# m96-chan/PyGPUkit

Hardware: AMD Instinct MI355X
Metric: decode tokens/sec/GPU + prefill TFLOPS (% MFMA peak), Qwen3-0.6B bf16 (higher is better)
Workload: dtype bf16

## Files before the change

### pygpukit_amd/csrc/engine.hip

```cpp

#include "engine_attn.hip.h"
#include "engine_gemv.hip.h"
#include "pkgemm.hip.h"

namespace pgk {

__global__ void embed_kernel(const bf16* embed, const int32_t* tokens, float* h, int H, const int32_t* positions,
                             const float* rope_cos, const float* rope_sin, float* cur_cos, float* cur_sin, int half,
                             int max_seq) {
    const int b = blockIdx.x;
    const bf16* row = embed + (size_t)tokens[b] * H;
    for (int i = threadIdx.x; i < H; i += blockDim.x) h[(size_t)b * H + i] = to_f(row[i]);
    const int pos = min(positions[b], max_seq - 1);
    for (int i = threadIdx.x; i < half; i += blockDim.x) {
        cur_cos[(size_t)b * half + i] = rope_cos[(size_t)pos * half + i];
        cur_sin[(size_t)b * half + i] = rope_sin[(size_t)pos * half + i];
    }
}

__global__ __launch_bounds__(256) void finalize_kernel(unsigned long long* tl, const float* amax_val, const int* amax_idx, int nblk,
                                                       int32_t* tokens, int32_t* positions, int32_t* token_log,
                                                       int32_t* step_counter, int log_width, int log_cap,
                                                       const bf16* embed, float* h, int H, int bump,
                                                       unsigned long long* clk_log, const float* rope_cos,
// ... 836 lines not shown
}

pgk_status pgk_engine_linear_plan(pgk_engine eh, int batch, int max_position, int prefill_n, char* out, size_t n) {
    PGK_REQUIRE(eh && out && n > 0, "pgk_engine_linear_plan: null argument");
    const Engine* e = (const Engine*)eh;
    const auto& c = e->cfg;
    size_t used = 0;
    out[0] = 0;
    auto emit = [&](const char* fmt, auto... args) -> bool {
        const int w = snprintf(out + used, n - used, fmt, args...);
        if (w <= 0 || (size_t)w >= n - used) return false;
        used += (size_t)w;
        return true;
    };
    const int H = c.hidden_size, I = c.intermediate_size, QD = c.num_heads * c.head_dim, NQKV = e->qkv_dim(), V = c.vocab_size;
    if (prefill_n > 0) {
        PGK_REQUIRE(prefill_n <= c.max_seq_len, "pgk_engine_linear_plan: %d tokens outside cache of %d", prefill_n, c.max_seq_len);
        const PrefillChoice p = prefill_choice(e, prefill_n);
        const char* path = p.fp8act ? "fp8act" : (p.pk ? "pk" : (p.ws ? "ws" : "gemm"));
        const int s_qkv = p.ws && !p.pk ? p.s_qkv : 1, s_gu = p.ws && !p.pk ? p.s_gu : 1;
        const int s_o = p.fp8act ? 1 : (p.pk ? (p.carried ? 1 : p.pk_so) : (p.ws ? p.s_o : p.g_so));
        const int s_d = p.fp8act ? 1 : (p.pk ? (p.carried ? 1 : p.pk_sd) : (p.ws ? p.s_d : p.g_sd));
        PGK_REQUIRE(emit("prefill n=%d path=%s ws=%d pk=%d pk_heads=%d carried=%d pkd=%d nvf4=%d fp8act=%d fuse_heads=%d fuse_heads8=%d fuse_sw16=%d fuse_sw8=%d "
                         "s_qkv=%d s_o=%d s_gu=%d s_d=%d\n", prefill_n, path, (int)p.ws, (int)p.pk, (int)p.pk_heads, (int)p.carried, (int)p.pkd, (int)p.nv4,
                         (int)p.fp8act, (int)p.fuse_heads, (int)p.fuse_heads8, (int)p.fuse_sw16, (int)p.fuse_sw8, s_qkv, s_o, s_gu, s_d),
                    "pgk_engine_linear_plan: the plan needs more than %zu bytes", n);
        return PGK_OK;
    }
    PGK_REQUIRE(batch >= 1 && batch <= c.max_batch, "pgk_engine_linear_plan: batch %d outside [1,%d]", batch, c.max_batch);
    PGK_REQUIRE(max_position >= 0 && max_position < c.max_seq_len, "pgk_engine_linear_plan: position %d outside cache of %d", max_position, c.max_seq_len);
    static const char* const forms[] = {"gemv", "batched", "tiled", "packed"};
    const bool short_ctx = step_is_short_at(e, batch, max_position) && e->short_path;
    const bool fp8 = c.weight_format == 1 || c.weight_format == 2;
    const int nw = c.weight_format == 3 ? GEMV_NW_NVF4 : (fp8 ? GEMV_NW_FP8 : GEMV_NW_BF16);
    const char* wname = c.weight_format == 3 ? "nvf4" : (fp8 ? "fp8" : "bf16");
    bool ok = true;
    for (int b0 = 0; b0 < batch && ok;) {
        const ChunkChoice ch = next_chunk(e, batch - b0);
        const AttnFlags af = attn_flags(e, ch.form, ch.m, short_ctx);
        const int M = ch.m;
        if (ch.form == CF_GEMV) {
            const bool partials = af.fused || af.merged;
            const char* act = M >= 4 ? "bf16" : "f32";
            ok = emit("chunk b0=%d m=%d form=gemv act=%s oproj=%s carried=0 normrows=0 attn16=none\n", b0, M, act, af.fused ? "fused" : (af.merged ? "merged" : "own"));
            auto gemv = [&](const char* name, int wnw, const char* wn, const char* pro, bool swiglu, int n_out, int K, int r, int force_grid) {
                if (r == 0) r = gemv_rows(wnw, M, swiglu, n_out, K);
                ok = ok && emit("proj name=%s kernel=fused_gemv m=%d act=%s w=%s pro=%s r=%d c=%d grid=%d n=%d k=%d\n", name, M, act, wn, pro, r,
                                gemv_preload(wnw, r, K), gemv_grid(r, swiglu, n_out, force_grid), n_out, K);
            };
            gemv("qkv", nw, wname, "norm", false, NQKV, H, 0, 0);
            if (!partials) gemv("o", nw, wname, "plain", false, H, QD, 0, 0);
            gemv("gate_up", nw, wname, partials && M <= 2 ? "norm_sum" : "norm", true, I, H, 0, 0);
            gemv("down", nw, wname, "plain", false, H, I, 0, 0);
            gemv("lm_head", GEMV_NW_BF16, "bf16", "norm", false, V, H, 4, e->lm_blocks);
        } else if (ch.form == CF_PACKED) {
            const bool carried = e->packed_resid;
            ok = emit("chunk b0=%d m=%d form=packed act=bf16 oproj=own carried=%d normrows=0 attn16=%s\n", b0, M, carried ? 1 : 0, af.direct ? "direct" : "normrows");
            ok = ok && emit("proj name=qkv kernel=pkgemm splits=1 n=%d k=%d\n", NQKV, H);
            ok = ok && emit("proj name=o kernel=%s splits=%d n=%d k=%d\n", carried ? "pkgemm_resid" : "pkgemm", carried ? 1 : pkgemm_pick_splits(M, H, QD), H, QD);
            ok = ok && emit("proj name=gate_up kernel=pkgemm splits=1 n=%d k=%d\n", 2 * I, H);
            ok = ok && emit("proj name=down kernel=%s splits=%d n=%d k=%d\n", carried ? "pkgemm_resid" : "pkgemm", carried ? 1 : pkgemm_pick_splits(M, H, I), H, I);
            const int rows = mt_rows_per_group(V, true);
            ok = ok && emit("proj name=lm_head kernel=batched_mt w=bf16 rows=%d mp=0 tiles=%d copy=%d grid=%d n=%d k=%d\n", rows, mt_tiles(M),
                            batched_reads_copy(false, rows, e->packed_lm != nullptr) ? 1 : 0, batched_lm_blocks(V), V, H);
        } else {
            const bool tiled = ch.form == CF_TILED;
            ok = emit("chunk b0=%d m=%d form=%s act=bf16 oproj=own carried=0 normrows=%d attn16=%s\n", b0, M, forms[ch.form], tiled ? 1 : 0,
                      af.direct ? "direct" : (tiled ? "normrows" : "none"));
            auto bat = [&](const char* name, bool wfp8, bool logits, bool have_copy, int N, int K) {
                const char* wn = wfp8 ? "fp8" : "bf16";
                if (tiled) {
                    const int rows = mt_rows_per_group(N, logits);
                    ok = ok && emit("proj name=%s kernel=batched_mt w=%s rows=%d mp=0 tiles=%d copy=%d grid=%d n=%d k=%d\n", name, wn, rows, mt_tiles(M),
                                    batched_reads_copy(wfp8, rows, have_copy) ? 1 : 0, logits ? batched_lm_blocks(V) : ceil_div(N, rows), N, K);
                } else if (batched_is_reg(K)) {
                    const int rows = batched_reg_rows(N, logits);
                    ok = ok && emit("proj name=%s kernel=batched_reg w=%s rows=%d mp=0 tiles=1 copy=%d grid=%d n=%d k=%d\n", name, wn, rows,
                                    batched_reads_copy(wfp8, rows, have_copy) ? 1 : 0, logits ? batched_lm_blocks(V) : ceil_div(N, rows), N, K);
                } else {
                    ok = ok && emit("proj name=%s kernel=batched_lds w=%s rows=16 mp=%d tiles=1 copy=0 grid=%d n=%d k=%d\n", name, wn, M <= 8 ? 8 : 16,
                                    logits ? batched_lm_blocks(V) : ceil_div(N, 16), N, K);
                }
            };
// ... 21 lines not shown
```

### pygpukit_amd/csrc/engine_prefill.hip

```cpp

#include "attn_plan.h"
#include "engine_gemv.hip.h"
#include "engine_state.hip.h"
#include "gemm_epilogues.hip.h"
#include "pkgemm.hip.h"

namespace pgk {

pgk_status engine_gemm_nt(const bf16* A, const void* W, const bf16* wscale, bool fp8, void* C, bool accum_f32, int M,
                          int N, int K, hipStream_t st, bool packed = false);
bool engine_gemm_packed_ok(int M, int N, int K);
int wsgemm_pick_splits(int N, int K, bool allow_split);
int engine_gemm_pick_splits(int M, int N, int K);
pgk_status engine_gemm_nt_slabs(const bf16* A, const void* W, float* slabs, int splits, int M, int N, int K, hipStream_t st, bool packed = false);
pgk_status gemm_fp8_nt(const uint8_t* a, const float* sa, const uint8_t* w, const bf16* sw, void* c, bool accum_f32, int M,
                       int N, int K, hipStream_t st);
pgk_status quantize_fp8_rows_bf16(const bf16* x, uint8_t* out, float* scale, int M, int K, hipStream_t st);
bool engine_gemm_qkv_heads_ok(int M, int N, int K);
pgk_status engine_gemm_qkv_heads_nt(const bf16* A, const bf16* W, bf16* qkv, int M, int N, int K, const QkvHeadArgs& hd, hipStream_t st, bool packed = false);
bool engine_gemm_swiglu_ok(int M, int I, int K, bool fp8);
pgk_status engine_gemm_swiglu_nt(const bf16* A, const void* W, const bf16* wscale, bool fp8, bf16* act, int M, int I, int K, hipStream_t st, bool packed = false);
bool gemm_fp8_qkv_heads_ok(int M, int N, int K);
pgk_status gemm_fp8_qkv_heads_nt(const uint8_t* a, const float* sa, const uint8_t* w, const bf16* sw, bf16* qkv, int M, int N, int K,
                                 const QkvHeadArgs& hd, hipStream_t st);
// ... 196 lines not shown
            *reinterpret_cast<uint2*>(q8 + s * I + c * 8) = o;
            if ((c & 15) == 0) q8s[s * (I >> 7) + (c >> 4)] = sc;
        } else {
            g.store(act + s * I + c * 8);
        }
    }
}

__global__ void bf16_rows_to_f32_kernel(const bf16* in, float* out, size_t n) {
    const size_t stride = (size_t)gridDim.x * blockDim.x;
    for (size_t i = blockIdx.x * (size_t)blockDim.x + threadIdx.x; i < n; i += stride) out[i] = to_f(in[i]);
}

pgk_status rmsnorm_slabs(float* h, const bf16* gamma, bf16* x, int rows, int H, float eps, const float* slabs, int* pending, uint8_t* q8,
                         float* q8s, hipStream_t st, int* launches) {
    const auto kfn = *pending <= 4 ? rmsnorm_f32_bf16_kernel<4> : rmsnorm_f32_bf16_kernel<16>;
    kfn<<<rows, 256, 0, st>>>(h, gamma, x, rows, H, eps, slabs, *pending, q8, q8s);
    *pending = 0;
    PGK_LAUNCH_CHECK();
    return counted(launches, PGK_OK);
}

pgk_status packed_mlp_carried(Engine* e, int layer, int rows, const bf16* attn16, bf16* act16, float* h, bf16* x16, int* ss_n, hipStream_t st,
                              int* launches) {
    const auto& c = e->cfg;
    const int H = c.hidden_size, I = c.intermediate_size, QD = c.num_heads * c.head_dim;
    const auto& P = e->packed[layer];
    if (pgk_status r = counted(launches, pkgemm_resid_nt(attn16, QD, P.o, h, rows, H, QD, (const bf16*)e->layers[layer].mlp_norm, x16, e->pk_ss, ss_n, st))) return r;
    mark(KC_GATEUP);
    PkArgs gn{};
    gn.ss_in = e->pk_ss; gn.ss_n = *ss_n; gn.ss_eps = c.norm_eps;
    if (pgk_status r = counted(launches, pkgemm_nt(x16, H, P.gate_up, act16, I, PK_EPI_SWIGLU, 1, rows, 2 * I, H, &gn, st))) return r;
    mark(KC_DOWN);
    const bf16* gnext = layer + 1 < c.num_layers ? (const bf16*)e->layers[layer + 1].attn_norm : nullptr;
    return counted(launches, pkgemm_resid_nt(act16, I, P.down, h, rows, H, I, gnext, x16, e->pk_ss, ss_n, st));
}

PrefillChoice prefill_choice(const Engine* e, int n) {
    const auto& c = e->cfg;
    const int H = c.hidden_size, I = c.intermediate_size, D = c.head_dim, QD = c.num_heads * D, NQKV = e->qkv_dim();
    PrefillChoice p{};
    const bool ws = p.ws = n <= 128;
    p.s_o = ws ? wsgemm_pick_splits(H, QD, true) : 1; p.s_d = ws ? wsgemm_pick_splits(H, I, true) : 1;
    p.s_qkv = ws ? wsgemm_pick_splits(NQKV, H, true) : 1; p.s_gu = ws ? wsgemm_pick_splits(2 * I, H, true) : 1;
    const bool pk = p.pk = ws && e->packed_ok;
    p.pk_so = pk ? pkgemm_pick_splits(n, H, QD) : 1; p.pk_sd = pk ? pkgemm_pick_splits(n, H, I) : 1;
    p.pk_heads = pk && D == 128;
    p.carried = pk && e->packed_resid;
    const bool pkd = p.pkd = !ws && c.weight_format == 1 && e->packed_have && engine_gemm_packed_ok(n, NQKV, H) && engine_gemm_packed_ok(n, H, QD) &&
                             engine_gemm_packed_ok(n, 2 * I, H) && engine_gemm_packed_ok(n, H, I);
    p.nv4 = c.weight_format == 3;
    const bool w16 = p.w16 = c.weight_format == 0 || p.nv4;
    const bool gsplit = p.gsplit = !ws && (w16 || pkd);
    p.g_so = gsplit ? engine_gemm_pick_splits(n, H, QD) : 1; p.g_sd = gsplit ? engine_gemm_pick_splits(n, H, I) : 1;
    const bool fp8 = p.fp8 = c.weight_format == 1 || c.weight_format == 2;
    const bool fp8act = p.fp8act = c.weight_format == 2 && n > 128;
    const bool fuse_epi = p.fuse_epi = env_on("PGK_FUSED_EPILOGUES");
    const bool fuse_q = p.fuse_q = fp8act && H % 128 == 0 && I % 128 == 0 && H <= 4096 && fuse_epi;
    p.fuse_sw8 = fuse_q && gemm_fp8_swiglu_ok(n, I, H);
    p.fuse_sw16 = !fp8act && !ws && fuse_epi && engine_gemm_swiglu_ok(n, I, H, fp8 && !pkd);
    p.fuse_heads8 = fuse_q && D == 128 && gemm_fp8_qkv_heads_ok(n, NQKV, H);
    p.fuse_heads = p.fuse_heads8 || (!ws && !pk && fuse_epi && (w16 || pkd) && D == 128 && engine_gemm_qkv_heads_ok(n, NQKV, H));
    return p;
}

template <class HeadArgs>
static void fill_head_args(HeadArgs& hd, const Engine* e, const pgk_layer_weights_t& L, bf16* kc, bf16* vc, int start_pos) {
    const auto& c = e->cfg;
    hd.q_gamma = c.use_qk_norm ? (const bf16*)L.q_norm : nullptr;
    hd.k_gamma = c.use_qk_norm ? (const bf16*)L.k_norm : nullptr;
    hd.eps = c.norm_eps; hd.rope_cos = e->rope_cos; hd.rope_sin = e->rope_sin; hd.kcache = kc; hd.vcache = vc;
    hd.hq = c.num_heads; hd.hkv = c.num_kv_heads; hd.max_seq = c.max_seq_len; hd.start_pos = start_pos;
}

}

using namespace pgk;

extern "C" {

pgk_status pgk_engine_prefill(pgk_engine eh, int seq, const int32_t* h_tokens, int n, int start_pos, void* all_logits,
                              float* h_last_logits, pgk_stream s) {
    PGK_REQUIRE(eh && h_tokens, "pgk_engine_prefill: null argument");
    Engine* e = (Engine*)eh;
    const auto& c = e->cfg;
    PGK_REQUIRE(seq >= 0 && seq < c.max_batch, "pgk_engine_prefill: sequence slot %d outside [0,%d)", seq, c.max_batch);
// ... 58 lines not shown
            const bool usep = pkd && wp != nullptr;
            const int gs = accum && gsplit ? engine_gemm_pick_splits(n, N_, K_) : 1;
            if (gs > 1) { pending = gs; return engine_gemm_nt_slabs(x_in, usep ? (const void*)wp : w, slabs, gs, n, N_, K_, st, usep); }
            if (usep) return engine_gemm_nt(x_in, wp, nullptr, false, dst, accum, n, N_, K_, st, true);
            return engine_gemm_nt(x_in, w, (const bf16*)sc, fp8, dst, accum, n, N_, K_, st);
        }
        if (splits == 1) return wsgemm_nt(x_in, K_, w, (const bf16*)sc, fp8, dst, nullptr, accum ? 2 : 0, 1, n, N_, K_, st);
        if (accum) pending = splits;
        return wsgemm_nt(x_in, K_, w, (const bf16*)sc, fp8, slabs, nullptr, 1, splits, n, N_, K_, st);
    };
    auto norm = [&](const bf16* gamma, bool to_fp8 = false) -> pgk_status {
        return rmsnorm_slabs(h32, gamma, x, n, H, c.norm_eps, slabs, &pending, to_fp8 ? q8 : nullptr, to_fp8 ? q8s : nullptr, st, nullptr);
    };
    if (ids_by_value) {
        EmbedTokenArgs ids{};
        for (int i = 0; i < n; ++i) ids.id[i] = h_tokens[i];
        embed_rows_arg_kernel<<<n, 256, 0, st>>>(e->embed, h32, H, ids);
    } else {
        embed_rows_kernel<<<n, 256, 0, st>>>(e->embed, e->pf_tokens, h32, H);
    }
    PGK_LAUNCH_CHECK();
    const int kv_len = start_pos + n;
    int ss_n = 0;
    for (int l = 0; l < c.num_layers; ++l) {
        pgk_layer_weights_t Lq = e->layers[l];
        if (nv4) {
            bf16* d = e->nv_deq;
            const struct { const void* w; const void* s; int N, K; } m4[4] = {
                {Lq.w_qkv, Lq.s_qkv, NQKV, H}, {Lq.w_o, Lq.s_o, H, QD}, {Lq.w_gate_up, Lq.s_gate_up, 2 * I, H}, {Lq.w_down, Lq.s_down, H, I}};
            const void** dst[4] = {&Lq.w_qkv, &Lq.w_o, &Lq.w_gate_up, &Lq.w_down};
            for (int i = 0; i < 4; ++i) {
                if (pgk_status r = dequant_nvf4_nk((const uint8_t*)m4[i].w, (const uint8_t*)m4[i].s, d, m4[i].N, m4[i].K, st)) return r;
                *dst[i] = d;
                d += (size_t)m4[i].N * m4[i].K;
            }
            Lq.s_qkv = Lq.s_o = Lq.s_gate_up = Lq.s_down = nullptr;
        }
        const auto& L = Lq;
        bf16* kc = e->kcache + (size_t)l * e->kv_layer_elems() + (size_t)seq * c.num_kv_heads * c.max_seq_len * D;
        bf16* vc = e->vcache + (size_t)l * e->kv_layer_elems() + (size_t)seq * c.num_kv_heads * c.max_seq_len * D;
        const bool carried = pc.carried;
        PkArgs nrm{};
        if (carried && l > 0) { nrm.ss_in = e->pk_ss; nrm.ss_n = ss_n; nrm.ss_eps = c.norm_eps; }
        else if (pgk_status r = norm((const bf16*)L.attn_norm, fuse_q)) return r;
        if (pk_heads) {
            PkArgs hd = nrm;
            fill_head_args(hd, e, L, kc, vc, start_pos);
            if (pgk_status r = pkgemm_nt(x, H, e->packed[l].qkv, qkv, NQKV, PK_EPI_QKV, 1, n, NQKV, H, &hd, st)) return r;
        } else if (pk) {
            if (pgk_status r = pkgemm_nt(x, H, e->packed[l].qkv, qkv, NQKV, PK_EPI_BF16, 1, n, NQKV, H, &nrm, st)) return r;
        } else if (fuse_heads) {
            QkvHeadArgs hd{};
            fill_head_args(hd, e, L, kc, vc, start_pos);
            if (fuse_heads8) {
                if (pgk_status r = gemm_fp8_qkv_heads_nt(q8, q8s, (const uint8_t*)L.w_qkv, (const bf16*)L.s_qkv, qkv, n, NQKV, H, hd, st)) return r;
            } else if (pgk_status r = engine_gemm_qkv_heads_nt(x, pkd ? e->packed[l].qkv : (const bf16*)L.w_qkv, qkv, n, NQKV, H, hd, st, pkd)) return r;
        } else {
            if (pgk_status r = proj(fuse_q ? nullptr : x, L.w_qkv, L.s_qkv, qkv, false, NQKV, H, s_qkv, pkd ? e->packed[l].qkv : nullptr)) return r;
        }
        if (!pk_heads && !fuse_heads) {
            const int s_qkv = pk ? 1 : s_qkv_ws;
            const int nslots = c.num_heads + 2 * c.num_kv_heads;
            const bf16* qg = c.use_qk_norm ? (const bf16*)L.q_norm : nullptr;
            const bf16* kg = c.use_qk_norm ? (const bf16*)L.k_norm : nullptr;
            const auto kfn = D == 128 ? qknorm_rope_kvwrite_kernel<128> : qknorm_rope_kvwrite_kernel<64>;
            kfn<<<ceil_div((long long)n * nslots, D == 128 ? 16 : 32), 256, 0, st>>>(
                qkv, qg, kg, c.norm_eps, e->rope_cos, e->rope_sin, kc, vc, n, c.num_heads, c.num_kv_heads, c.max_seq_len, start_pos, slabs,
                s_qkv > 1 ? s_qkv : 0);
            PGK_LAUNCH_CHECK();
        }
        const bool attn_q8 = fuse_q && D == 128 && n > 128 && sdpa_flash_enabled();
        if (attn_q8) {
            if (pgk_status r = flash_prefill_q8(qkv, kc, vc, q8, q8s, c.num_heads, c.num_kv_heads, n, kv_len, 1.0f / sqrtf((float)D), D, NQKV,
                                                (long long)c.max_seq_len * D, D, st))
                return r;
        } else if (pgk_status r = pgk_sdpa_causal(qkv, kc, vc, attn, c.num_heads, c.num_kv_heads, n, kv_len, D, 0.f, D, NQKV,
                                                  (int64_t)c.max_seq_len * D, D, D, QD, PGK_BF16, st))
            return r;
        auto pk_accum = [&](const bf16* x_in, const bf16* wp, int K_, int splits) -> pgk_status {
            if (splits == 1) return pkgemm_nt(x_in, K_, wp, h32, H, PK_EPI_ACCUM, 1, n, H, K_, nullptr, st);
            pending = splits;
            return pkgemm_nt(x_in, K_, wp, slabs, H, PK_EPI_SLAB, splits, n, H, K_, nullptr, st);
        };
        if (carried) {
            if (pgk_status r = packed_mlp_carried(e, l, n, attn, act, h32, x, &ss_n, st, nullptr)) return r;
            continue;
        }
        if (pk) { if (pgk_status r = pk_accum(attn, e->packed[l].o, QD, pk_so)) return r; }
        else if (pgk_status r = proj(attn_q8 ? nullptr : attn, L.w_o, L.s_o, h32, true, H, QD, s_o, pkd ? e->packed[l].o : nullptr)) return r;
        if (pgk_status r = norm((const bf16*)L.mlp_norm, fuse_q)) return r;
        if (pk) {
            if (pgk_status r = pkgemm_nt(x, H, e->packed[l].gate_up, act, I, PK_EPI_SWIGLU, 1, n, 2 * I, H, nullptr, st)) return r;
            if (pgk_status r = pk_accum(act, e->packed[l].down, I, pk_sd)) return r;
            continue;
        }
        if (fuse_sw8) {
            if (pgk_status r = gemm_fp8_swiglu_nt(q8, q8s, (const uint8_t*)L.w_gate_up, (const bf16*)L.s_gate_up, q8b, q8bs, n, I, H, st)) return r;
            if (pgk_status r = gemm_fp8_nt(q8b, q8bs, (const uint8_t*)L.w_down, (const bf16*)L.s_down, h32, true, n, H, I, st)) return r;
            continue;
        }
        if (fuse_sw16) {
            if (pgk_status r = engine_gemm_swiglu_nt(x, pkd ? (const void*)e->packed[l].gate_up : L.w_gate_up, (const bf16*)L.s_gate_up, fp8 && !pkd, act, n, I, H, st, pkd)) return r;
            if (pgk_status r = proj(act, L.w_down, L.s_down, h32, true, H, I, s_d, pkd ? e->packed[l].down : nullptr)) return r;
            continue;
        }
        if (pgk_status r = proj(fuse_q ? nullptr : x, L.w_gate_up, L.s_gate_up, gu, false, 2 * I, H, s_gu, pkd ? e->packed[l].gate_up : nullptr)) return r;
        swiglu_rows_kernel<<<ceil_div((long long)n * I / 8, 256) > 2048 ? 2048 : ceil_div((long long)n * I / 8, 256), 256, 0, st>>>(
            gu, act, n, I, slabs, s_gu > 1 ? s_gu : 0, fuse_q ? q8 : nullptr, fuse_q ? q8s : nullptr);
        PGK_LAUNCH_CHECK();
        if (pgk_status r = proj(fuse_q ? nullptr : act, L.w_down, L.s_down, h32, true, H, I, s_d, pkd ? e->packed[l].down : nullptr)) return r;
    }
    if (pgk_status r = norm(e->final_norm)) return r;
    if (all_logits) {
        if (pgk_status r = engine_gemm_nt(x, e->lm_head, nullptr, false, all_logits, false, n, c.vocab_size, H, st)) return r;
    }
    if (h_last_logits) {
        float* xin = h32;
        bf16_rows_to_f32_kernel<<<4, 256, 0, st>>>(x + (size_t)(n - 1) * H, xin, H);
        PGK_LAUNCH_CHECK();
        FusedArgs a{};
        a.w = e->lm_head; a.N = c.vocab_size; a.K = H; a.xin = xin;
        a.out = e->logits + (size_t)seq * c.vocab_size; a.ld_out = c.vocab_size;
        if (pgk_status r = launch_fused<bf16, float, 1, 4, PRO_PLAIN, EPI_STORE>(a, c.vocab_size, st)) return r;
        PGK_CHECK_HIP(hipMemcpyAsync(h_last_logits, a.out, (size_t)c.vocab_size * 4, hipMemcpyDeviceToHost, st));
        PGK_CHECK_HIP(hipStreamSynchronize(st));
    }
    return PGK_OK;
}

}
```

### pygpukit_amd/csrc/engine_state.hip.h

```cpp
#pragma once

#include <algorithm>
#include <cstdlib>
#include <type_traits>
#include <vector>

#include "engine_common.hip.h"

namespace pgk {

constexpr int SHORT_CTX = 512;
constexpr int SHORT_CTX_B1 = 384;

struct Engine {
    pgk_model_config_t cfg;
    const bf16 *embed, *lm_head, *final_norm;
    std::vector<pgk_layer_weights_t> layers;
    int nsplit = 1, lm_blocks = 1, lm_cap = 1, log_cap = 4096;
    bool batched_mfma = true;
    int batched_min = 5, batched_max = 64;
    int cu_count = 256;
    bool short_path = true;
    int pos_hi = -1;
    float sample_temperature = 0.f, sample_top_p = 1.f;
// ... 131 lines not shown
}

inline bool batched_is_reg(int K) { const int s = K / 128; return s == 8 || s == 16 || s == 24 || s == 32; }
inline int batched_reg_rows(int N, bool logits) { return (logits || (N + 15) / 16 >= 192) ? 16 : ((N + 7) / 8 >= 192 ? 8 : 4); }
inline int mt_rows_per_group(int N, bool logits) { return (logits || (N + 15) / 16 >= 192) ? 16 : 4; }
inline int mt_tiles(int M) { return M <= 32 ? 2 : 4; }
inline bool batched_reads_copy(bool fp8, int rows_per_group, bool have_copy) { return !fp8 && rows_per_group == 16 && have_copy; }
inline bool batched_layer_copy(const Engine* e, bool fp8) { return !fp8 && e->packed_ok; }
inline int batched_lm_blocks(int vocab) { const int g = (vocab + 15) / 16; return g < 2048 ? g : 2048; }

struct PrefillChoice {
    bool ws;
    bool pk;
    bool pk_heads;
    bool carried;
    bool pkd;
    bool nv4, w16, gsplit, fp8, fp8act;
    bool fuse_epi, fuse_q, fuse_sw8, fuse_sw16, fuse_heads8, fuse_heads;
    int s_o, s_d, s_qkv, s_gu;
    int pk_so, pk_sd;
    int g_so, g_sd;
};
PrefillChoice prefill_choice(const Engine* e, int n);

pgk_status rmsnorm_slabs(float* h, const bf16* gamma, bf16* x, int rows, int H, float eps, const float* slabs, int* pending, uint8_t* q8,
                         float* q8s, hipStream_t st, int* launches);
pgk_status packed_mlp_carried(Engine* e, int layer, int rows, const bf16* attn16, bf16* act16, float* h, bf16* x16, int* ss_n, hipStream_t st,
                              int* launches);

}
```

### pygpukit_amd/csrc/ops_pkgemm.hip

```cpp

#include "gemv_core.hip.h"
#include "pgk_internal.h"
#include "pkgemm.hip.h"

namespace pgk {

typedef __bf16 bf16x8_p __attribute__((ext_vector_type(8)));
typedef float f32x4_p __attribute__((ext_vector_type(4)));

constexpr int PK_THREADS = 256;
constexpr int PK_MT = 2;
constexpr int PK_MB = PK_MT * 16;
constexpr int PK_RING = 16;

__device__ __forceinline__ void pk_dma16(const void* src, uint32_t lds_addr) {
    asm volatile("s_mov_b32 m0, %1\n\ts_nop 0\n\tglobal_load_lds_dwordx4 %0, off" ::"v"(src), "s"(lds_addr) : "memory", "m0");
}
__device__ __forceinline__ uint32_t pk_lds_addr(const char* p) {
    return (uint32_t)(uintptr_t)(__attribute__((address_space(3))) const char*)p;
}
__device__ __forceinline__ int pk_swz(int c, int row) { return (c & ~15) | ((c ^ row) & 15); }

__global__ void pack_weights_kernel(const bf16* w, bf16* wp, int N, int K) {
    const size_t chunks = (size_t)N * K / 8, stride = (size_t)gridDim.x * blockDim.x;
// ... 29 lines not shown
        const f32x2 c0 = __builtin_amdgcn_cvt_pk_f32_fp8((int)v.x, false), c1 = __builtin_amdgcn_cvt_pk_f32_fp8((int)v.x, true);
        const f32x2 c2 = __builtin_amdgcn_cvt_pk_f32_fp8((int)v.y, false), c3 = __builtin_amdgcn_cvt_pk_f32_fp8((int)v.y, true);
        *reinterpret_cast<uint4*>(wp + t * 8) = make_uint4(pack_bf16x2(c0.x * sc, c0.y * sc), pack_bf16x2(c1.x * sc, c1.y * sc),
                                                          pack_bf16x2(c2.x * sc, c2.y * sc), pack_bf16x2(c3.x * sc, c3.y * sc));
    }
}

pgk_status pack_weights_fp8(const void* w, const void* scale, void* wp, int N, int K, hipStream_t st) {
    PGK_REQUIRE(N % 16 == 0 && K % 128 == 0 && scale != nullptr, "pack_weights_fp8: N=%d must be a multiple of 16, K=%d of 128, scales present", N, K);
    const size_t chunks = (size_t)N * K / 8;
    const int grid = (int)(chunks / 256 > 4096 ? 4096 : (chunks + 255) / 256);
    pack_weights_fp8_kernel<<<grid, 256, 0, st>>>((const uint8_t*)w, (const bf16*)scale, (bf16*)wp, N, K);
    PGK_CHECK_HIP(hipGetLastError());
    return PGK_OK;
}

#ifdef PGK_PHASE_STAMPS
__device__ unsigned long long g_pk_stamps[5][512][8];
#define PK_STAMP(i) do { if (threadIdx.x == 0 && blockIdx.x < 512) g_pk_stamps[EPI][blockIdx.x][i] = __builtin_amdgcn_s_memrealtime(); } while (0)
#else
#define PK_STAMP(i) do { } while (0)
#endif

template <int NTW, int EPI, int MT>
__global__ __launch_bounds__(PK_THREADS) void pkgemm_kernel(PkArgs g) {
    constexpr int PK_MT = MT, PK_MB = 16 * MT;
    extern __shared__ __attribute__((aligned(16))) char a_lds[];
    __shared__ float ssred[4][PK_MB];
    PK_STAMP(0);
    const int lane = threadIdx.x & 63, wid = __builtin_amdgcn_readfirstlane(threadIdx.x >> 6);
    const int l15 = lane & 15, q = lane >> 4;
    int cb, mb, sp;
    {
        const int per = 8 * g.mblk * g.splits;
        const int grp = blockIdx.x / per, r = blockIdx.x - grp * per;
        cb = grp * 8 + (r & 7);
        int rest = r >> 3;
        mb = rest % g.mblk;
        sp = rest / g.mblk;
        if (cb >= g.nblk) return;
    }
    const int m0 = mb * PK_MB;
    const int ks0 = sp * g.ksteps, KS = g.ksteps, ksn = g.K / 32;
    const int rb = KS * 64;
    const int tile_a = cb * g.tiles_per_cb + wid;
    const bf16* wrun[NTW];
    wrun[0] = g.wp + ((size_t)tile_a * ksn + ks0) * 512 + lane * 8;
    if constexpr (NTW == 2) wrun[1] = g.wp + ((size_t)(tile_a + g.tile_b_off) * ksn + ks0) * 512 + lane * 8;

    __shared__ __attribute__((aligned(16))) float rope_lds[EPI == PK_EPI_QKV ? 2 * PK_MB * 64 : 4];
    uint16_t gbits[2] = {0, 0};
    bool is_q = false, is_k = false, has_gamma = false;
    if constexpr (EPI == PK_EPI_QKV) {
        is_q = cb < g.hq;
        is_k = !is_q && cb < g.hq + g.hkv;
        const int d = 16 * wid + l15;
        const bf16* gm = is_q ? g.q_gamma : g.k_gamma;
        has_gamma = gm != nullptr && (is_q || is_k);
        const bf16* gsafe = has_gamma ? gm : reinterpret_cast<const bf16*>(g.rope_cos);
        gbits[0] = gsafe[d].bits; gbits[1] = gsafe[d + 64].bits;
        if (is_q || is_k) {
            const uint32_t r0 = pk_lds_addr(reinterpret_cast<const char*>(rope_lds));
            constexpr int IPT = PK_MB / 4;
            for (int j = wid; j < 2 * IPT; j += 4) {
                const int row = 4 * (j % IPT) + q;
                const int pos = min(g.start_pos + min(m0 + row, g.M - 1), g.max_seq - 1);
                pk_dma16(((j / IPT) ? g.rope_sin : g.rope_cos) + (size_t)pos * 64 + 4 * l15, r0 + j * 1024);
            }
        }
    }

    __shared__ float inv_lds[PK_MB];
    const bool scaled = g.ss_in != nullptr;
    float4 ssu, ssv;
    {
        const int row = threadIdx.x >> 3, sub = threadIdx.x & 7;
        const float* sp = scaled ? g.ss_in + (size_t)min(m0 + min(row, PK_MB - 1), g.M - 1) * PK_SS_LD + 8 * sub
                                 : reinterpret_cast<const float*>(g.wp) + 8 * sub;
        ssu = *reinterpret_cast<const float4*>(sp);
        ssv = *reinterpret_cast<const float4*>(sp + 4);
    }
    {
        const uint32_t lds0 = pk_lds_addr(a_lds);
        const int ndma = PK_MB * rb / 1024, gpr = KS >> 2;
        const uint32_t magic = (65536u + gpr - 1) / gpr;
        const bf16* abase = g.a + (size_t)ks0 * 32;
        for (int j = wid; j < ndma; j += 4) {
            const int grp = 4 * j + q;
            const int row = (int)(((uint32_t)grp * magic) >> 16), gi = grp - row * gpr;
            const int c = gi * 16 + ((l15 ^ row) & 15);
            pk_dma16(abase + (size_t)min(m0 + row, g.M - 1) * g.lda + c * 8, lds0 + j * 1024);
        }
    }
    uint4 wr[NTW][PK_RING];
#pragma unroll
    for (int s = 0; s < PK_RING; ++s)
#pragma unroll
        for (int t = 0; t < NTW; ++t) wr[t][s] = *reinterpret_cast<const uint4*>(wrun[t] + (size_t)min(s, KS - 1) * 512);
    if (scaled) {
        const int row = threadIdx.x >> 3, sub = threadIdx.x & 7;
        const float p8[8] = {ssu.x, ssu.y, ssu.z, ssu.w, ssv.x, ssv.y, ssv.z, ssv.w};
        float ssum = 0.f;
#pragma unroll
        for (int i = 0; i < 8; ++i) ssum += (8 * sub + i < g.ss_n) ? p8[i] : 0.f;
        ssum = group8_sum(ssum);
        if (sub == 0 && row < PK_MB) inv_lds[row] = 1.0f / sqrtf(ssum / (float)g.K + g.ss_eps);
    }
    PK_STAMP(1);
    if constexpr (NTW == 2) asm volatile("s_waitcnt vmcnt(32)" ::: "memory");
    else asm volatile("s_waitcnt vmcnt(16)" ::: "memory");
    __syncthreads();
    PK_STAMP(2);

    f32x4_p acc[NTW][PK_MT];
#pragma unroll
    for (int t = 0; t < NTW; ++t)
#pragma unroll
        for (int mt = 0; mt < PK_MT; ++mt) acc[t][mt] = f32x4_p{0.f, 0.f, 0.f, 0.f};

    uint4 af[4][PK_MT];
    int aoff[PK_MT][4];
#pragma unroll
    for (int mt = 0; mt < PK_MT; ++mt)
#pragma unroll
        for (int j = 0; j < 4; ++j) aoff[mt][j] = (mt * 16 + l15) * rb + ((((4 * j + q) ^ l15) & 15) << 4);
    auto read_a = [&](int ks, int j, uint4 (&dst)[PK_MT]) {
#pragma unroll
        for (int mt = 0; mt < PK_MT; ++mt) dst[mt] = *reinterpret_cast<const uint4*>(a_lds + aoff[mt][j] + ((ks >> 2) << 8));
    };
// ... 291 lines not shown
            for (int mt = 0; mt < MT; ++mt) mine[(t * MT + mt) * 64] = make_float4(acc[t][mt][0], acc[t][mt][1], acc[t][mt][2], acc[t][mt][3]);
    }
    __syncthreads();
    const float* kp = reinterpret_cast<const float*>(kpart);
#pragma unroll
    for (int i = 0; i < EPT; ++i) {
        const int m = em[i], n = en[i];
        const int idx = ((((n >> 4) * MT + (m >> 4)) * 64) + 16 * ((m & 15) >> 2) + (n & 15)) * 4 + (m & 3);
        float v = hold[i];
        v += (kp[idx] + kp[idx + NTW * MT * 256]) + (kp[idx + 2 * NTW * MT * 256] + kp[idx + 3 * NTW * MT * 256]);
        const bool ok = m0 + m < g.M;
        if (ok) g.h[(size_t)(m0 + m) * g.N + n0 + n] = v;
        if (g.gamma_next) {
            if (ok) g.xpre[(size_t)(m0 + m) * g.N + n0 + n] = from_f<bf16>(v * bf16_bits_to_f(gnb[i]));
            const float sq = group_sum<NC>(v * v);
            if (n == 0 && ok) g.ss_out[(size_t)(m0 + m) * PK_SS_LD + cb] = sq;
        }
    }
}

bool pkgemm_resid_ok(int N, int K) { return N % 32 == 0 && N / 16 <= PK_SS_LD && K % 512 == 0 && 16 * (K / 32) * 64 <= 128 * 1024; }

pgk_status pkgemm_resid_nt(const bf16* a, int lda, const void* wp, float* h, int M, int N, int K, const bf16* gamma_next, bf16* xpre,
                           float* ss_out, int* ss_n, hipStream_t st) {
    PGK_REQUIRE(M >= 1 && M <= 128 && pkgemm_resid_ok(N, K) && lda % 8 == 0, "pkgemm_resid: M=%d N=%d K=%d lda=%d not supported", M, N, K, lda);
    PGK_REQUIRE(!gamma_next || (xpre && ss_out && ss_n), "pkgemm_resid: the next norm's outputs are missing");
    PkResidArgs g{a, lda, (const bf16*)wp, M, N, K, 0, 0, h, gamma_next, xpre, ss_out};
    const bool small = (N / 16) * ceil_div(M, 16) <= 256;
    const bool wide = !small && (size_t)32 * (K / 32) * 64 <= 128 * 1024;
    const int mb = wide ? 32 : 16, ntw = (small || wide) ? 1 : 2;
    g.nblk = N / (16 * ntw);
    g.mblk = ceil_div(M, mb);
    if (ss_n) *ss_n = g.nblk;
    const size_t lds = (size_t)mb * (K / 32) * 64;
    const int grid = ceil_div(g.nblk, 8) * 8 * g.mblk;
#define PGK_PKR_LAUNCH(MBV, NTWV)                                                                                  \
    {                                                                                                              \
        static bool attr = false;                                                                                  \
        if (lds > 48 * 1024 && !attr) {                                                                            \
            PGK_CHECK_HIP(hipFuncSetAttribute(reinterpret_cast<const void*>(&pkgemm_resid_kernel<MBV, NTWV>),       \
                                              hipFuncAttributeMaxDynamicSharedMemorySize, (int)(128 * 1024)));     \
            attr = true;                                                                                           \
        }                                                                                                          \
        pkgemm_resid_kernel<MBV, NTWV><<<grid, PK_THREADS, lds, st>>>(g);                                          \
    }
    if (small) PGK_PKR_LAUNCH(16, 1) else if (wide) PGK_PKR_LAUNCH(32, 1) else PGK_PKR_LAUNCH(16, 2)
#undef PGK_PKR_LAUNCH
    PGK_CHECK_HIP(hipGetLastError());
    return PGK_OK;
}

int pkgemm_pick_splits(int M, int N, int K) {
    const int nblk = N / 64, mblk = ceil_div(M, M <= 96 ? 16 : 32);
    int best = 0;
    for (int s = 1; s <= 16; ++s) {
        if (K % (s * 128) != 0 || K / s > 2048) continue;
        best = s;
        if (nblk * mblk * s >= 256) break;
    }
    return best;
}

bool pkgemm_shape_ok(int N, int K, bool splittable) {
    return N % 64 == 0 && K % 128 == 0 && (splittable ? pkgemm_pick_splits(128, N, K) > 0 : K <= 2048);
}

pgk_status pkgemm_nt(const bf16* a, int lda, const void* wp, void* c, int ldc, int epi, int splits, int M, int N, int K, const PkArgs* head,
                     hipStream_t st) {
    PGK_REQUIRE(M >= 1 && M <= 128, "pkgemm: M=%d outside [1,128]", M);
    PGK_REQUIRE(N % 64 == 0 && K % 128 == 0 && lda % 8 == 0, "pkgemm: N=%d K=%d lda=%d not supported", N, K, lda);
    PGK_REQUIRE(splits >= 1 && K % (splits * 128) == 0 && (epi == PK_EPI_SLAB || splits == 1), "pkgemm: %d K-splits not usable here", splits);
    PkArgs g = head ? *head : PkArgs{};
    g.a = a; g.lda = lda; g.wp = (const bf16*)wp; g.M = M; g.N = N; g.K = K; g.c = c; g.ldc = ldc;
    g.ksteps = K / splits / 32;
    g.splits = splits;
    g.tiles_per_cb = 4;
    g.tile_b_off = 0;
    if (epi == PK_EPI_SWIGLU) {
        PGK_REQUIRE(N % 128 == 0, "pkgemm: SwiGLU needs 2 I = %d weight rows with I a multiple of 64", N);
        g.nblk = N / 2 / 64;
        g.tile_b_off = N / 2 / 16;
    } else if (epi == PK_EPI_QKV) {
        PGK_REQUIRE(head && N == (g.hq + 2 * g.hkv) * 128, "pkgemm: head epilogue needs head_dim 128 (N=%d)", N);
        g.nblk = N / 128;
        g.tiles_per_cb = 8;
        g.tile_b_off = 4;
    } else {
        g.nblk = N / 64;
    }
    const int mt = (M <= 96 || g.nblk * splits * ceil_div(M, 16) <= 256) ? 1 : 2;
    g.mblk = ceil_div(M, 16 * mt);
    const size_t lds = (size_t)16 * mt * g.ksteps * 64;
    PGK_REQUIRE(lds <= 128 * 1024, "pkgemm: K per workgroup %d too long for the LDS activation block", g.ksteps * 32);
    const int grid = ceil_div(g.nblk, 8) * 8 * g.mblk * splits;
#define PGK_PK_LAUNCH2(NTWV, EPIV, MTV)                                                                            \
    {                                                                                                              \
        static size_t attr = 0;                                                                                    \
        if (lds > 48 * 1024 && lds > attr) {                                                                       \
            PGK_CHECK_HIP(hipFuncSetAttribute(reinterpret_cast<const void*>(&pkgemm_kernel<NTWV, EPIV, MTV>),       \
                                              hipFuncAttributeMaxDynamicSharedMemorySize, (int)(128 * 1024)));     \
            attr = 128 * 1024;                                                                                     \
        }                                                                                                          \
        pkgemm_kernel<NTWV, EPIV, MTV><<<grid, PK_THREADS, lds, st>>>(g);                                          \
    }
#define PGK_PK_LAUNCH(NTWV, EPIV)                                                                                  \
    if (mt == 1) PGK_PK_LAUNCH2(NTWV, EPIV, 1) else PGK_PK_LAUNCH2(NTWV, EPIV, 2)
    switch (epi) {
        case PK_EPI_BF16: PGK_PK_LAUNCH(1, PK_EPI_BF16) break;
        case PK_EPI_SLAB: PGK_PK_LAUNCH(1, PK_EPI_SLAB) break;
        case PK_EPI_ACCUM: PGK_PK_LAUNCH(1, PK_EPI_ACCUM) break;
        case PK_EPI_SWIGLU: PGK_PK_LAUNCH(2, PK_EPI_SWIGLU) break;
        case PK_EPI_QKV: PGK_PK_LAUNCH(2, PK_EPI_QKV) break;
        default: return set_error(PGK_ERR_INVALID, "pkgemm: unknown epilogue %d", epi);
    }
#undef PGK_PK_LAUNCH2
#undef PGK_PK_LAUNCH
    PGK_CHECK_HIP(hipGetLastError());
    return PGK_OK;
}

}
```

### pygpukit_amd/csrc/pkgemm.hip.h

```cpp
#pragma once

#include "pgk_device.hip.h"
#include "pgk_internal.h"

namespace pgk {

enum { PK_EPI_BF16 = 0, PK_EPI_SLAB = 1, PK_EPI_ACCUM = 2, PK_EPI_SWIGLU = 3, PK_EPI_QKV = 4 };

struct PkArgs {
    const bf16* a;
    int lda;
    const bf16* wp;
    int M, N, K;
    int ksteps;
    int nblk, mblk, splits;
    int tiles_per_cb;
    int tile_b_off;
    void* c;
    int ldc;
    const bf16 *q_gamma, *k_gamma;
    float eps;
    const float *rope_cos, *rope_sin;
    bf16 *kcache, *vcache;
    int hq, hkv, max_seq, start_pos;
    const float* ss_in;
    int ss_n;
    float ss_eps;
};

constexpr int PK_SS_LD = 64;

pgk_status pack_weights_bf16(const void* w, void* wp, int N, int K, hipStream_t st);
pgk_status pack_weights_fp8(const void* w, const void* scale, void* wp, int N, int K, hipStream_t st);
int pkgemm_pick_splits(int M, int N, int K);
bool pkgemm_shape_ok(int N, int K, bool splittable);
bool pkgemm_resid_ok(int N, int K);
pgk_status pkgemm_resid_nt(const bf16* a, int lda, const void* wp, float* h, int M, int N, int K, const bf16* gamma_next, bf16* xpre,
                           float* ss_out, int* ss_n, hipStream_t st);
pgk_status pkgemm_nt(const bf16* a, int lda, const void* wp, void* c, int ldc, int epi, int splits, int M, int N, int K, const PkArgs* head,
                     hipStream_t st);

}
```

Baseline: 1700.

## Compute only the last-token tail in final prefill layer; add 3-wave SwiGLU pkgemm

In the last layer of prefill, when only last-token logits are needed and the packed carried path is active, attention, o-proj, MLP and final norm run only on the trailing row tile, not all n rows. This removes most of the final layer's work, which is not needed for the requested output. The resid GEMM keeps the tile choice it would make for the full row count so numerics match. Separately, the SwiGLU pkgemm gains a 3-wave, 48-column-block variant, picked when its workgroup count lands closer to the CU count, to improve wave quantization on the gate_up projection.

```diff
diff --git a/pygpukit_amd/csrc/engine.hip b/pygpukit_amd/csrc/engine.hip
--- a/pygpukit_amd/csrc/engine.hip
+++ b/pygpukit_amd/csrc/engine.hip
@@ -882,8 +882,10 @@
         const int s_o = p.fp8act ? 1 : (p.pk ? (p.carried ? 1 : p.pk_so) : (p.ws ? p.s_o : p.g_so));
         const int s_d = p.fp8act ? 1 : (p.pk ? (p.carried ? 1 : p.pk_sd) : (p.ws ? p.s_d : p.g_sd));
         PGK_REQUIRE(emit("prefill n=%d path=%s ws=%d pk=%d pk_heads=%d carried=%d pkd=%d nvf4=%d fp8act=%d fuse_heads=%d fuse_heads8=%d fuse_sw16=%d fuse_sw8=%d "
-                         "s_qkv=%d s_o=%d s_gu=%d s_d=%d\n", prefill_n, path, (int)p.ws, (int)p.pk, (int)p.pk_heads, (int)p.carried, (int)p.pkd, (int)p.nv4,
-                         (int)p.fp8act, (int)p.fuse_heads, (int)p.fuse_heads8, (int)p.fuse_sw16, (int)p.fuse_sw8, s_qkv, s_o, s_gu, s_d),
+                         "s_qkv=%d s_o=%d s_gu=%d s_d=%d gu_waves=%d tail_last=%d tail_none=%d\n", prefill_n, path, (int)p.ws, (int)p.pk, (int)p.pk_heads,
+                         (int)p.carried, (int)p.pkd, (int)p.nv4, (int)p.fp8act, (int)p.fuse_heads, (int)p.fuse_heads8, (int)p.fuse_sw16, (int)p.fuse_sw8, s_qkv,
+                         s_o, s_gu, s_d, p.pk ? pkgemm_swiglu_waves(prefill_n, I) : 0, prefill_tail_rows(e, p, prefill_n, prefill_n, false, true),
+                         prefill_tail_rows(e, p, prefill_n, prefill_n, false, false)),
                     "pgk_engine_linear_plan: the plan needs more than %zu bytes", n);
         return PGK_OK;
     }
@@ -918,7 +920,7 @@
             ok = emit("chunk b0=%d m=%d form=packed act=bf16 oproj=own carried=%d normrows=0 attn16=%s\n", b0, M, carried ? 1 : 0, af.direct ? "direct" : "normrows");
             ok = ok && emit("proj name=qkv kernel=pkgemm splits=1 n=%d k=%d\n", NQKV, H);
             ok = ok && emit("proj name=o kernel=%s splits=%d n=%d k=%d\n", carried ? "pkgemm_resid" : "pkgemm", carried ? 1 : pkgemm_pick_splits(M, H, QD), H, QD);
-            ok = ok && emit("proj name=gate_up kernel=pkgemm splits=1 n=%d k=%d\n", 2 * I, H);
+            ok = ok && emit("proj name=gate_up kernel=pkgemm splits=1 waves=%d n=%d k=%d\n", pkgemm_swiglu_waves(M, I), 2 * I, H);
             ok = ok && emit("proj name=down kernel=%s splits=%d n=%d k=%d\n", carried ? "pkgemm_resid" : "pkgemm", carried ? 1 : pkgemm_pick_splits(M, H, I), H, I);
             const int rows = mt_rows_per_group(V, true);
             ok = ok && emit("proj name=lm_head kernel=batched_mt w=bf16 rows=%d mp=0 tiles=%d copy=%d grid=%d n=%d k=%d\n", rows, mt_tiles(M),
diff --git a/pygpukit_amd/csrc/engine_prefill.hip b/pygpukit_amd/csrc/engine_prefill.hip
--- a/pygpukit_amd/csrc/engine_prefill.hip
+++ b/pygpukit_amd/csrc/engine_prefill.hip
@@ -1,3 +1,5 @@
+
+#include <cstring>
 
 #include "attn_plan.h"
 #include "engine_gemv.hip.h"
@@ -242,18 +244,18 @@
 }
 
 pgk_status packed_mlp_carried(Engine* e, int layer, int rows, const bf16* attn16, bf16* act16, float* h, bf16* x16, int* ss_n, hipStream_t st,
-                              int* launches) {
+                              int* launches, int plan_rows) {
     const auto& c = e->cfg;
     const int H = c.hidden_size, I = c.intermediate_size, QD = c.num_heads * c.head_dim;
     const auto& P = e->packed[layer];
-    if (pgk_status r = counted(launches, pkgemm_resid_nt(attn16, QD, P.o, h, rows, H, QD, (const bf16*)e->layers[layer].mlp_norm, x16, e->pk_ss, ss_n, st))) return r;
+    if (pgk_status r = counted(launches, pkgemm_resid_nt(attn16, QD, P.o, h, rows, H, QD, (const bf16*)e->layers[layer].mlp_norm, x16, e->pk_ss, ss_n, st, plan_rows))) return r;
     mark(KC_GATEUP);
     PkArgs gn{};
     gn.ss_in = e->pk_ss; gn.ss_n = *ss_n; gn.ss_eps = c.norm_eps;
     if (pgk_status r = counted(launches, pkgemm_nt(x16, H, P.gate_up, act16, I, PK_EPI_SWIGLU, 1, rows, 2 * I, H, &gn, st))) return r;
     mark(KC_DOWN);
     const bf16* gnext = layer + 1 < c.num_layers ? (const bf16*)e->layers[layer + 1].attn_norm : nullptr;
-    return counted(launches, pkgemm_resid_nt(act16, I, P.down, h, rows, H, I, gnext, x16, e->pk_ss, ss_n, st));
+    return counted(launches, pkgemm_resid_nt(act16, I, P.down, h, rows, H, I, gnext, x16, e->pk_ss, ss_n, st, plan_rows));
 }
 
 PrefillChoice prefill_choice(const Engine* e, int n) {
@@ -282,6 +284,21 @@
     p.fuse_heads8 = fuse_q && D == 128 && gemm_fp8_qkv_heads_ok(n, NQKV, H);
     p.fuse_heads = p.fuse_heads8 || (!ws && !pk && fuse_epi && (w16 || pkd) && D == 128 && engine_gemm_qkv_heads_ok(n, NQKV, H));
     return p;
+}
+
+int prefill_tail_rows(const Engine* e, const PrefillChoice& pc, int n, int kv_len, bool all_logits, bool last_logits) {
+    const char* tv = getenv("PGK_PREFILL_TAIL");
+    if ((tv && strcmp(tv, "full") == 0) || all_logits) return n;
+    if (!last_logits) return 0;
+    const auto& c = e->cfg;
+    if (!(pc.pk && pc.pk_heads && pc.carried)) return n;
+    const int D = c.head_dim;
+    const FlashStrides sd{D, e->qkv_dim(), (long long)c.max_seq_len * D, D, D, (long long)c.num_heads * D};
+    const bool flash_on = sdpa_flash_enabled();
+    const int tn = n - ((n - 1) / 32) * 32;
+    const bool one_tile = sdpa_causal_pick(true, true, D, n, kv_len, true, true, sd, flash_on) == SDPA_ONE_TILE &&
+                          sdpa_causal_pick(true, true, D, tn, kv_len, true, true, sd, flash_on) == SDPA_ONE_TILE;
+    return one_tile ? tn : n;
 }
 
 template <class HeadArgs>
@@ -386,7 +403,10 @@
     PGK_LAUNCH_CHECK();
     const int kv_len = start_pos + n;
     int ss_n = 0;
+    const int tn = prefill_tail_rows(e, pc, n, kv_len, all_logits != nullptr, h_last_logits != nullptr), t0 = n - tn;
     for (int l = 0; l < c.num_layers; ++l) {
+        const bool last = l + 1 == c.num_layers;
+        const int r0 = last ? t0 : 0, rn = n - r0;
         pgk_layer_weights_t Lq = e->layers[l];
         if (nv4) {
             bf16* d = e->nv_deq;
@@ -433,13 +453,14 @@
                 s_qkv > 1 ? s_qkv : 0);
             PGK_LAUNCH_CHECK();
         }
+        if (rn == 0) break;
         const bool attn_q8 = fuse_q && D == 128 && n > 128 && sdpa_flash_enabled();
         if (attn_q8) {
             if (pgk_status r = flash_prefill_q8(qkv, kc, vc, q8, q8s, c.num_heads, c.num_kv_heads, n, kv_len, 1.0f / sqrtf((float)D), D, NQKV,
                                                 (long long)c.max_seq_len * D, D, st))
                 return r;
-        } else if (pgk_status r = pgk_sdpa_causal(qkv, kc, vc, attn, c.num_heads, c.num_kv_heads, n, kv_len, D, 0.f, D, NQKV,
-                                                  (int64_t)c.max_seq_len * D, D, D, QD, PGK_BF16, st))
+        } else if (pgk_status r = pgk_sdpa_causal(qkv + (size_t)r0 * NQKV, kc, vc, attn + (size_t)r0 * QD, c.num_heads, c.num_kv_heads, rn, kv_len, D, 0.f, D,
+                                                  NQKV, (int64_t)c.max_seq_len * D, D, D, QD, PGK_BF16, st))
             return r;
         auto pk_accum = [&](const bf16* x_in, const bf16* wp, int K_, int splits) -> pgk_status {
             if (splits == 1) return pkgemm_nt(x_in, K_, wp, h32, H, PK_EPI_ACCUM, 1, n, H, K_, nullptr, st);
@@ -447,7 +468,9 @@
             return pkgemm_nt(x_in, K_, wp, slabs, H, PK_EPI_SLAB, splits, n, H, K_, nullptr, st);
         };
         if (carried) {
-            if (pgk_status r = packed_mlp_carried(e, l, n, attn, act, h32, x, &ss_n, st, nullptr)) return r;
+            if (pgk_status r = packed_mlp_carried(e, l, rn, attn + (size_t)r0 * QD, act + (size_t)r0 * I, h32 + (size_t)r0 * H, x + (size_t)r0 * H, &ss_n, st,
+                                                  nullptr, n))
+                return r;
             continue;
         }
         if (pk) { if (pgk_status r = pk_accum(attn, e->packed[l].o, QD, pk_so)) return r; }
@@ -474,7 +497,8 @@
         PGK_LAUNCH_CHECK();
         if (pgk_status r = proj(fuse_q ? nullptr : act, L.w_down, L.s_down, h32, true, H, I, s_d, pkd ? e->packed[l].down : nullptr)) return r;
     }
-    if (pgk_status r = norm(e->final_norm)) return r;
+    if (tn == 0) return PGK_OK;
+    if (pgk_status r = rmsnorm_slabs(h32 + (size_t)t0 * H, e->final_norm, x + (size_t)t0 * H, tn, H, c.norm_eps, slabs, &pending, nullptr, nullptr, st, nullptr)) return r;
     if (all_logits) {
         if (pgk_status r = engine_gemm_nt(x, e->lm_head, nullptr, false, all_logits, false, n, c.vocab_size, H, st)) return r;
     }
diff --git a/pygpukit_amd/csrc/engine_state.hip.h b/pygpukit_amd/csrc/engine_state.hip.h
--- a/pygpukit_amd/csrc/engine_state.hip.h
+++ b/pygpukit_amd/csrc/engine_state.hip.h
@@ -177,10 +177,11 @@
     int g_so, g_sd;
 };
 PrefillChoice prefill_choice(const Engine* e, int n);
+int prefill_tail_rows(const Engine* e, const PrefillChoice& pc, int n, int kv_len, bool all_logits, bool last_logits);
 
 pgk_status rmsnorm_slabs(float* h, const bf16* gamma, bf16* x, int rows, int H, float eps, const float* slabs, int* pending, uint8_t* q8,
                          float* q8s, hipStream_t st, int* launches);
 pgk_status packed_mlp_carried(Engine* e, int layer, int rows, const bf16* attn16, bf16* act16, float* h, bf16* x16, int* ss_n, hipStream_t st,
-                              int* launches);
+                              int* launches, int plan_rows = 0);
 
 }
diff --git a/pygpukit_amd/csrc/ops_pkgemm.hip b/pygpukit_amd/csrc/ops_pkgemm.hip
--- a/pygpukit_amd/csrc/ops_pkgemm.hip
+++ b/pygpukit_amd/csrc/ops_pkgemm.hip
@@ -75,8 +75,9 @@
 #define PK_STAMP(i) do { } while (0)
 #endif
 
-template <int NTW, int EPI, int MT>
-__global__ __launch_bounds__(PK_THREADS) void pkgemm_kernel(PkArgs g) {
+template <int NTW, int EPI, int MT, int NWV = 4>
+__global__ __launch_bounds__(64 * NWV) void pkgemm_kernel(PkArgs g) {
+    static_assert(NWV == 4 || (NWV == 3 && EPI == PK_EPI_SWIGLU), "three waves: the SwiGLU epilogue only");
     constexpr int PK_MT = MT, PK_MB = 16 * MT;
     extern __shared__ __attribute__((aligned(16))) char a_lds[];
     __shared__ float ssred[4][PK_MB];
@@ -115,7 +116,7 @@
         if (is_q || is_k) {
             const uint32_t r0 = pk_lds_addr(reinterpret_cast<const char*>(rope_lds));
             constexpr int IPT = PK_MB / 4;
-            for (int j = wid; j < 2 * IPT; j += 4) {
+            for (int j = wid; j < 2 * IPT; j += NWV) {
                 const int row = 4 * (j % IPT) + q;
                 const int pos = min(g.start_pos + min(m0 + row, g.M - 1), g.max_seq - 1);
                 pk_dma16(((j / IPT) ? g.rope_sin : g.rope_cos) + (size_t)pos * 64 + 4 * l15, r0 + j * 1024);
@@ -125,20 +126,22 @@
 
     __shared__ float inv_lds[PK_MB];
     const bool scaled = g.ss_in != nullptr;
-    float4 ssu, ssv;
-    {
-        const int row = threadIdx.x >> 3, sub = threadIdx.x & 7;
+    constexpr int SS_RPP = 8 * NWV, SS_PASSES = (PK_MB + SS_RPP - 1) / SS_RPP;
+    float4 ssu[SS_PASSES], ssv[SS_PASSES];
+#pragma unroll
+    for (int ps = 0; ps < SS_PASSES; ++ps) {
+        const int row = (threadIdx.x >> 3) + ps * SS_RPP, sub = threadIdx.x & 7;
         const float* sp = scaled ? g.ss_in + (size_t)min(m0 + min(row, PK_MB - 1), g.M - 1) * PK_SS_LD + 8 * sub
                                  : reinterpret_cast<const float*>(g.wp) + 8 * sub;
-        ssu = *reinterpret_cast<const float4*>(sp);
-        ssv = *reinterpret_cast<const float4*>(sp + 4);
+        ssu[ps] = *reinterpret_cast<const float4*>(sp);
+        ssv[ps] = *reinterpret_cast<const float4*>(sp + 4);
     }
     {
         const uint32_t lds0 = pk_lds_addr(a_lds);
         const int ndma = PK_MB * rb / 1024, gpr = KS >> 2;
         const uint32_t magic = (65536u + gpr - 1) / gpr;
         const bf16* abase = g.a + (size_t)ks0 * 32;
-        for (int j = wid; j < ndma; j += 4) {
+        for (int j = wid; j < ndma; j += NWV) {
             const int grp = 4 * j + q;
             const int row = (int)(((uint32_t)grp * magic) >> 16), gi = grp - row * gpr;
             const int c = gi * 16 + ((l15 ^ row) & 15);
@@ -151,13 +154,16 @@
 #pragma unroll
         for (int t = 0; t < NTW; ++t) wr[t][s] = *reinterpret_cast<const uint4*>(wrun[t] + (size_t)min(s, KS - 1) * 512);
     if (scaled) {
-        const int row = threadIdx.x >> 3, sub = threadIdx.x & 7;
-        const float p8[8] = {ssu.x, ssu.y, ssu.z, ssu.w, ssv.x, ssv.y, ssv.z, ssv.w};
-        float ssum = 0.f;
-#pragma unroll
-        for (int i = 0; i < 8; ++i) ssum += (8 * sub + i < g.ss_n) ? p8[i] : 0.f;
-        ssum = group8_sum(ssum);
-        if (sub == 0 && row < PK_MB) inv_lds[row] = 1.0f / sqrtf(ssum / (float)g.K + g.ss_eps);
+#pragma unroll
+        for (int ps = 0; ps < SS_PASSES; ++ps) {
+            const int row = (threadIdx.x >> 3) + ps * SS_RPP, sub = threadIdx.x & 7;
+            const float p8[8] = {ssu[ps].x, ssu[ps].y, ssu[ps].z, ssu[ps].w, ssv[ps].x, ssv[ps].y, ssv[ps].z, ssv[ps].w};
+            float ssum = 0.f;
+#pragma unroll
+            for (int i = 0; i < 8; ++i) ssum += (8 * sub + i < g.ss_n) ? p8[i] : 0.f;
+            ssum = group8_sum(ssum);
+            if (sub == 0 && row < PK_MB) inv_lds[row] = 1.0f / sqrtf(ssum / (float)g.K + g.ss_eps);
+        }
     }
     PK_STAMP(1);
     if constexpr (NTW == 2) asm volatile("s_waitcnt vmcnt(32)" ::: "memory");
@@ -495,11 +501,12 @@
 bool pkgemm_resid_ok(int N, int K) { return N % 32 == 0 && N / 16 <= PK_SS_LD && K % 512 == 0 && 16 * (K / 32) * 64 <= 128 * 1024; }
 
 pgk_status pkgemm_resid_nt(const bf16* a, int lda, const void* wp, float* h, int M, int N, int K, const bf16* gamma_next, bf16* xpre,
-                           float* ss_out, int* ss_n, hipStream_t st) {
+                           float* ss_out, int* ss_n, hipStream_t st, int plan_m) {
     PGK_REQUIRE(M >= 1 && M <= 128 && pkgemm_resid_ok(N, K) && lda % 8 == 0, "pkgemm_resid: M=%d N=%d K=%d lda=%d not supported", M, N, K, lda);
+    if (plan_m < M) plan_m = M;
     PGK_REQUIRE(!gamma_next || (xpre && ss_out && ss_n), "pkgemm_resid: the next norm's outputs are missing");
     PkResidArgs g{a, lda, (const bf16*)wp, M, N, K, 0, 0, h, gamma_next, xpre, ss_out};
-    const bool small = (N / 16) * ceil_div(M, 16) <= 256;
+    const bool small = (N / 16) * ceil_div(plan_m, 16) <= 256;
     const bool wide = !small && (size_t)32 * (K / 32) * 64 <= 128 * 1024;
     const int mb = wide ? 32 : 16, ntw = (small || wide) ? 1 : 2;
     g.nblk = N / (16 * ntw);
@@ -538,6 +545,15 @@
     return N % 64 == 0 && K % 128 == 0 && (splittable ? pkgemm_pick_splits(128, N, K) > 0 : K <= 2048);
 }
 
+int pkgemm_swiglu_waves(int M, int I) {
+    const int tiles = I / 16;
+    const char* wv = getenv("PGK_PK_WAVES");
+    if (tiles % 3 != 0 || (wv && atoi(wv) == 4)) return 4;
+    const int cus = device_cu_count();
+    auto wgs = [&](int nblk) { return nblk * ceil_div(M, (M <= 96 || nblk * ceil_div(M, 16) <= 256) ? 16 : 32); };
+    return abs(wgs(tiles / 3) - cus) < abs(wgs(tiles / 4) - cus) ? 3 : 4;
+}
+
 pgk_status pkgemm_nt(const bf16* a, int lda, const void* wp, void* c, int ldc, int epi, int splits, int M, int N, int K, const PkArgs* head,
                      hipStream_t st) {
     PGK_REQUIRE(M >= 1 && M <= 128, "pkgemm: M=%d outside [1,128]", M);
@@ -549,10 +565,16 @@
     g.splits = splits;
     g.tiles_per_cb = 4;
     g.tile_b_off = 0;
+    int waves = 4;
     if (epi == PK_EPI_SWIGLU) {
         PGK_REQUIRE(N % 128 == 0, "pkgemm: SwiGLU needs 2 I = %d weight rows with I a multiple of 64", N);
         g.nblk = N / 2 / 64;
         g.tile_b_off = N / 2 / 16;
+        waves = pkgemm_swiglu_waves(M, N / 2);
+        if (waves == 3) {
+            g.nblk = N / 2 / 48;
+            g.tiles_per_cb = 3;
+        }
     } else if (epi == PK_EPI_QKV) {
         PGK_REQUIRE(head && N == (g.hq + 2 * g.hkv) * 128, "pkgemm: head epilogue needs head_dim 128 (N=%d)", N);
         g.nblk = N / 128;
@@ -566,23 +588,26 @@
     const size_t lds = (size_t)16 * mt * g.ksteps * 64;
     PGK_REQUIRE(lds <= 128 * 1024, "pkgemm: K per workgroup %d too long for the LDS activation block", g.ksteps * 32);
     const int grid = ceil_div(g.nblk, 8) * 8 * g.mblk * splits;
-#define PGK_PK_LAUNCH2(NTWV, EPIV, MTV)                                                                            \
+#define PGK_PK_LAUNCH2(NTWV, EPIV, MTV, NWVV)                                                                          \
     {                                                                                                              \
         static size_t attr = 0;                                                                                    \
         if (lds > 48 * 1024 && lds > attr) {                                                                       \
-            PGK_CHECK_HIP(hipFuncSetAttribute(reinterpret_cast<const void*>(&pkgemm_kernel<NTWV, EPIV, MTV>),       \
+            PGK_CHECK_HIP(hipFuncSetAttribute(reinterpret_cast<const void*>(&pkgemm_kernel<NTWV, EPIV, MTV, NWVV>), \
                                               hipFuncAttributeMaxDynamicSharedMemorySize, (int)(128 * 1024)));     \
             attr = 128 * 1024;                                                                                     \
         }                                                                                                          \
-        pkgemm_kernel<NTWV, EPIV, MTV><<<grid, PK_THREADS, lds, st>>>(g);                                          \
+        pkgemm_kernel<NTWV, EPIV, MTV, NWVV><<<grid, 64 * NWVV, lds, st>>>(g);                                     \
     }
 #define PGK_PK_LAUNCH(NTWV, EPIV)                                                                                  \
-    if (mt == 1) PGK_PK_LAUNCH2(NTWV, EPIV, 1) else PGK_PK_LAUNCH2(NTWV, EPIV, 2)
+    if (mt == 1) PGK_PK_LAUNCH2(NTWV, EPIV, 1, 4) else PGK_PK_LAUNCH2(NTWV, EPIV, 2, 4)
     switch (epi) {
         case PK_EPI_BF16: PGK_PK_LAUNCH(1, PK_EPI_BF16) break;
         case PK_EPI_SLAB: PGK_PK_LAUNCH(1, PK_EPI_SLAB) break;
         case PK_EPI_ACCUM: PGK_PK_LAUNCH(1, PK_EPI_ACCUM) break;
-        case PK_EPI_SWIGLU: PGK_PK_LAUNCH(2, PK_EPI_SWIGLU) break;
+        case PK_EPI_SWIGLU:
+            if (waves == 3) { if (mt == 1) PGK_PK_LAUNCH2(2, PK_EPI_SWIGLU, 1, 3) else PGK_PK_LAUNCH2(2, PK_EPI_SWIGLU, 2, 3) }
+            else PGK_PK_LAUNCH(2, PK_EPI_SWIGLU)
+            break;
         case PK_EPI_QKV: PGK_PK_LAUNCH(2, PK_EPI_QKV) break;
         default: return set_error(PGK_ERR_INVALID, "pkgemm: unknown epilogue %d", epi);
     }
diff --git a/pygpukit_amd/csrc/pkgemm.hip.h b/pygpukit_amd/csrc/pkgemm.hip.h
--- a/pygpukit_amd/csrc/pkgemm.hip.h
+++ b/pygpukit_amd/csrc/pkgemm.hip.h
@@ -33,10 +33,11 @@
 pgk_status pack_weights_bf16(const void* w, void* wp, int N, int K, hipStream_t st);
 pgk_status pack_weights_fp8(const void* w, const void* scale, void* wp, int N, int K, hipStream_t st);
 int pkgemm_pick_splits(int M, int N, int K);
+int pkgemm_swiglu_waves(int M, int I);
 bool pkgemm_shape_ok(int N, int K, bool splittable);
 bool pkgemm_resid_ok(int N, int K);
 pgk_status pkgemm_resid_nt(const bf16* a, int lda, const void* wp, float* h, int M, int N, int K, const bf16* gamma_next, bf16* xpre,
-                           float* ss_out, int* ss_n, hipStream_t st);
+                           float* ss_out, int* ss_n, hipStream_t st, int plan_m = 0);
 pgk_status pkgemm_nt(const bf16* a, int lda, const void* wp, void* c, int ldc, int epi, int splits, int M, int N, int K, const PkArgs* head,
                      hipStream_t st);
 
```

After: 1699, median of 2. Within noise of the previous version (-0.1%).
